# yuanming-hu/exposure

Measured on AMD Instinct MI355X. Metric: Mpixels/s through 8-step filter chain fwd+bwd, higher is better.
Workload: dtype f16; 1 GPU; 8-step filter chain (E,G,W,S+,T,Ct,BW,C) fwd+bwd, 64x512x512x3 f16 NHWC per GPU, one HIP kernel per filter step and direction; batch_per_gpu=64, global_batch=64, height=512, width=512, parallelism=image-sharded replicas x1 (no data-path collective), weak scaling, launch=hipGraph replay, 10 steps (330 captured launches) per replay, chain_streams=2, transport=none (one process)

## Files before the change

exposure_amd/csrc/exposure_hip.hip:

```cpp
#include <dlfcn.h>
#include <hip/hip_runtime.h>
#include <stdint.h>
#include <stdio.h>
#include <stdlib.h>
#include <string.h>
#include <mutex>
#include <vector>
#include <string>
#include <type_traits>

#include "../../include/exposure_hip.h"
#include "filter_math.h"
#include "pixel_io.h"
#include "kernel_common.h"
#include "host_common.h"
#include "stream_bodies.h"



namespace expo {


template <class F, typename T, bool VEC, class IO>
__global__ __launch_bounds__(kThreads) void filter_fwd_kernel(const T* __restrict__ x, T* __restrict__ y,
// ... 1388 lines not shown
  if (g.stream) hipLaunchKernelGGL((vignet_fwd_kernel<T, true, IoStream>), grid, block, 0, s, (const T*)x, (T*)y, mp, sharp, masking, h, w, g.groups);
  else if (g.vec) hipLaunchKernelGGL((vignet_fwd_kernel<T, true>), grid, block, 0, s, (const T*)x, (T*)y, mp, sharp, masking, h, w, g.groups);
  else hipLaunchKernelGGL((vignet_fwd_kernel<T, false>), grid, block, 0, s, (const T*)x, (T*)y, mp, sharp, masking, h, w, g.groups);
  HIP_TRY(hipGetLastError(), "vignet_fwd launch");
  return EXPO_OK;
}

template <typename T>
static int vignet_bwd_t(const void* x, const void* dy, void* dx, const float* mp, float* dmp, float sharp, int masking,
                        int n, int h, int w, void* workspace, size_t workspace_bytes, hipStream_t s) {
  const Geom g = make_geom<T>(n, h, w, {x, dy, dx}, kGeomApply);
  const dim3 grid(g.blocks_x, n), block(kThreads);
  float* records;
  if (int rc = ws_check(workspace, workspace_bytes, n, g.blocks_x, 1, &records)) return rc;
#define EXPO_L(VEC, HAS_DX, IO) \
  hipLaunchKernelGGL((vignet_bwd_kernel<T, VEC, HAS_DX, IO>), grid, block, 0, s, (const T*)x, (const T*)dy, (T*)dx, mp, records, sharp, masking, h, w, g.groups)
  if (g.vec) { if (dx) EXPO_L(true, true, IoCached); else EXPO_L(true, false, IoCached); }
  else { if (dx) EXPO_L(false, true, IoCached); else EXPO_L(false, false, IoCached); }
#undef EXPO_L
  HIP_TRY(hipGetLastError(), "vignet_bwd launch");
  FinishArgs fa{};
  fa.s[0] = FinishStep{mp, dmp, nullptr, records, nullptr, kFinVignet, 0, masking ? 1 : 0, sharp, g.blocks_x};
  return launch_finish(fa, 1, n, s);
}

template <typename T>
static int penalty_bwd_t(const void* y, const float* dpen, void* dy, int n, int h, int w, hipStream_t s) {
  const Geom g = make_geom<T>(n, h, w, {y, dy}, kGeomMap);
  const dim3 grid(g.blocks_x, n), block(kThreads);
  const float inv_count = 1.0f / (float(g.hw) * 3.0f);
#define EXPO_L(VEC, IO) \
  hipLaunchKernelGGL((penalty_bwd_kernel<T, VEC, IO>), grid, block, 0, s, (const T*)y, dpen, (T*)dy, g.hw, g.groups, inv_count)
  if (g.stream) EXPO_L(true, IoStream); else if (g.vec) EXPO_L(true, IoCached); else EXPO_L(false, IoCached);
#undef EXPO_L
  HIP_TRY(hipGetLastError(), "penalty_bwd launch");
  return EXPO_OK;
}

template <typename T>
static int stats_bwd_t(const void* x, const float* stats, const float* dstats, void* dx, int n, int h, int w,
                       hipStream_t s) {
  const Geom g = make_geom<T>(n, h, w, {x, dx}, kGeomMap);
  const dim3 grid(g.blocks_x, n), block(kThreads);
  const float inv_hw = 1.0f / float(g.hw);
#define EXPO_L(VEC, IO) \
  hipLaunchKernelGGL((stats_bwd_kernel<T, VEC, IO>), grid, block, 0, s, (const T*)x, stats, dstats, (T*)dx, g.hw, g.groups, inv_hw)
  if (g.stream) EXPO_L(true, IoStream); else if (g.vec) EXPO_L(true, IoCached); else EXPO_L(false, IoCached);
#undef EXPO_L
  HIP_TRY(hipGetLastError(), "stats_bwd launch");
  return EXPO_OK;
}

template <typename T>
static int stats_jvp_t(const void* x, const float* stats, const void* v, float* jv, int n, int h, int w,
                       void* workspace, size_t workspace_bytes, hipStream_t s) {
  const Geom g = make_geom<T>(n, h, w, {x, v}, kGeomReadReduce);
  const dim3 grid(g.blocks_x, n), block(kThreads);
  float* records;
  if (int rc = ws_check(workspace, workspace_bytes, n, g.blocks_x, 1, &records)) return rc;
#define EXPO_L(VEC, IO) \
  hipLaunchKernelGGL((stats_jvp_kernel<T, VEC, IO>), grid, block, 0, s, (const T*)x, stats, (const T*)v, records, g.hw, g.groups)
  if (g.stream) EXPO_L(true, IoStream); else if (g.vec) EXPO_L(true, IoCached); else EXPO_L(false, IoCached);
#undef EXPO_L
  HIP_TRY(hipGetLastError(), "stats_jvp launch");
  FinishArgs fa{};
  fa.s[0] = FinishStep{nullptr, jv, nullptr, records, nullptr, kFinScaled, 3, 0, 1.0f / float(g.hw), g.blocks_x};
  return launch_finish(fa, 1, n, s);
}

template <typename T>
static int stats_hvp_t(const void* x, const float* dstats, const float* jv, const void* v, void* out, int n, int h,
                       int w, hipStream_t s) {
  const Geom g = make_geom<T>(n, h, w, {x, v, out}, kGeomMap);
  const dim3 grid(g.blocks_x, n), block(kThreads);
  const float inv_hw = 1.0f / float(g.hw);
#define EXPO_L(VEC, IO) \
  hipLaunchKernelGGL((stats_hvp_kernel<T, VEC, IO>), grid, block, 0, s, (const T*)x, dstats, jv, (const T*)v, (T*)out, g.hw, g.groups, inv_hw)
  if (g.stream) EXPO_L(true, IoStream); else if (g.vec) EXPO_L(true, IoCached); else EXPO_L(false, IoCached);
#undef EXPO_L
  HIP_TRY(hipGetLastError(), "stats_hvp launch");
  return EXPO_OK;
}

}

using namespace expo;

struct ForkJoin {
  hipStream_t helper = nullptr;
  hipEvent_t fork = nullptr, join = nullptr;
};
__device__ int g_lane_probe[2];
__global__ void lane_probe_wait_kernel(int gen, long long limit_ticks) {
  if (threadIdx.x != 0) return;
  const long long t0 = wall_clock64();
  int seen = 0;
  do {
    seen = __hip_atomic_load(&g_lane_probe[0], __ATOMIC_RELAXED, __HIP_MEMORY_SCOPE_AGENT);
    if (seen == gen) break;
    __builtin_amdgcn_s_sleep(64);
  } while (wall_clock64() - t0 < limit_ticks);
  __hip_atomic_store(&g_lane_probe[1], seen == gen ? gen : -gen, __ATOMIC_RELAXED, __HIP_MEMORY_SCOPE_AGENT);
}
__global__ void lane_probe_set_kernel(int gen) {
  if (threadIdx.x == 0) __hip_atomic_store(&g_lane_probe[0], gen, __ATOMIC_RELAXED, __HIP_MEMORY_SCOPE_AGENT);
}
static int lanes_run_side_by_side(hipStream_t s, hipStream_t h) {
  static int gen = 0;
  ++gen;
  hipLaunchKernelGGL(lane_probe_wait_kernel, dim3(1), dim3(64), 0, s, gen, 50000LL);
  hipLaunchKernelGGL(lane_probe_set_kernel, dim3(1), dim3(64), 0, h, gen);
  if (hipGetLastError() != hipSuccess) return -1;
  if (hipStreamSynchronize(h) != hipSuccess || hipStreamSynchronize(s) != hipSuccess) return -1;
  int got[2] = {0, 0};
  if (hipMemcpyFromSymbol(got, HIP_SYMBOL(g_lane_probe), sizeof(got)) != hipSuccess) return -1;
  return got[1] == gen ? 1 : got[1] == -gen ? 0 : -1;
}
static int g_helper_probes = 0, g_helper_rejected = 0;

constexpr int kMaxProbeAttempts = 4;
constexpr size_t kMaxSpares = 8;
struct HelperEntry {
  int dev;
  hipStream_t caller;
  unsigned long long caller_id;
  ForkJoin fj;
  bool probed;
  std::mutex mu;
};
static std::vector<HelperEntry*> g_helper_table;
static std::vector<hipStream_t> g_helper_spares;
static std::mutex g_helper_mu;
static bool helper_probe_enabled() {
  static const bool probe = !(getenv("EXPO_CHAIN_HELPER_PROBE") && atoi(getenv("EXPO_CHAIN_HELPER_PROBE")) == 0);
  return probe;
}
static unsigned long long stream_id_of(hipStream_t s) {
  using GetId = hipError_t (*)(hipStream_t, unsigned long long*);
  static const GetId get_id = reinterpret_cast<GetId>(dlsym(RTLD_DEFAULT, "hipStreamGetId"));
  unsigned long long id = 0;
  if (!get_id) return 0;
  if (get_id(s, &id) != hipSuccess) {
    (void)hipGetLastError();
    id = 0;
  }
  return id;
}
static void park_or_destroy(hipStream_t st) {
  std::lock_guard<std::mutex> lock(g_helper_mu);
  if (g_helper_spares.size() < kMaxSpares)
    g_helper_spares.push_back(st);
  else
    (void)hipStreamDestroy(st);
}
static void probe_helper(HelperEntry* e) {
  hipStreamCaptureMode mode = hipStreamCaptureModeRelaxed;
  (void)hipThreadExchangeStreamCaptureMode(&mode);
  hipStream_t first = e->fj.helper, cand = first;
  bool found = false;
  for (int attempt = 0; attempt < kMaxProbeAttempts; ++attempt) {
    {
      std::lock_guard<std::mutex> lock(g_helper_mu);
      ++g_helper_probes;
    }
    const int r = lanes_run_side_by_side(e->caller, cand);
    if (r != 0) {
      found = true;
      break;
    }
    {
      std::lock_guard<std::mutex> lock(g_helper_mu);
      ++g_helper_rejected;
    }
    if (cand != first) park_or_destroy(cand);
    cand = nullptr;
    if (attempt + 1 == kMaxProbeAttempts) break;
    if (hipStreamCreateWithFlags(&cand, hipStreamNonBlocking) != hipSuccess) {
      (void)hipGetLastError();
      cand = nullptr;
      break;
    }
  }
  if (found && cand != first) {
    park_or_destroy(first);
    e->fj.helper = cand;
  }
  (void)hipThreadExchangeStreamCaptureMode(&mode);
  e->probed = true;
}

static HelperEntry* helper_entry(hipStream_t caller, bool probe_now) {
  int dev = 0;
  if (hipGetDevice(&dev) != hipSuccess || dev < 0) return nullptr;
  const unsigned long long id = stream_id_of(caller);
  HelperEntry* e = nullptr;
  {
    std::lock_guard<std::mutex> lock(g_helper_mu);
    for (HelperEntry* t : g_helper_table)
      if (t->dev == dev && t->caller == caller) e = t;
    if (e && e->caller_id != id) {
      e->caller_id = id;
      e->probed = !helper_probe_enabled();
    }
    if (!e) {
      hipStream_t st;
      hipEvent_t e0, e1;
      if (hipStreamCreateWithFlags(&st, hipStreamNonBlocking) != hipSuccess) return nullptr;
      if (hipEventCreateWithFlags(&e0, hipEventDisableTiming) != hipSuccess ||
          hipEventCreateWithFlags(&e1, hipEventDisableTiming) != hipSuccess) return nullptr;
      e = new HelperEntry{dev, caller, id, ForkJoin{st, e0, e1}, !helper_probe_enabled(), {}};
      g_helper_table.push_back(e);
    }
  }
  if (!probe_now) return e;
  std::lock_guard<std::mutex> lock(e->mu);
  if (e->probed) return e;
  hipStreamCaptureStatus cap = hipStreamCaptureStatusNone;
  if (hipStreamIsCapturing(caller, &cap) != hipSuccess) {
    (void)hipGetLastError();
    return e;
  }
  if (cap != hipStreamCaptureStatusNone) return e;
  probe_helper(e);
  return e;
}
static ForkJoin* fork_join_for_device(hipStream_t caller = nullptr) {
  HelperEntry* e = helper_entry(caller, true);
  return e ? &e->fj : nullptr;
}
static std::mutex g_fork_join_mu;
static int chain_fork(ForkJoin* fj, hipStream_t s) {
  std::lock_guard<std::mutex> lock(g_fork_join_mu);
  HIP_TRY(hipEventRecord(fj->fork, s), "chain fork");
  HIP_TRY(hipStreamWaitEvent(fj->helper, fj->fork, 0), "chain fork");
  return EXPO_OK;
}
static int chain_join(ForkJoin* fj, hipStream_t s) {
  std::lock_guard<std::mutex> lock(g_fork_join_mu);
  HIP_TRY(hipEventRecord(fj->join, fj->helper), "chain join");
  HIP_TRY(hipStreamWaitEvent(s, fj->join, 0), "chain join");
  return EXPO_OK;
}
static bool chain_split(int n, int h, int w, int dtype) {
  static const int forced = getenv("EXPO_CHAIN_STREAMS") ? atoi(getenv("EXPO_CHAIN_STREAMS")) : 0;
  if (n < 2) return false;
  if (forced == 1) return false;
  if (forced >= 2) return true;
  const long bytes = long(n) * h * w * 3L * (dtype == EXPO_F16 ? 2L : 4L);
  return bytes >= (40L << 20) && bytes < (256L << 20);
}

static bool chain_snake(int n, int h, int w, int dtype) {
  static const int forced = getenv("EXPO_CHAIN_SNAKE") ? atoi(getenv("EXPO_CHAIN_SNAKE")) : -1;
  if (forced >= 0) return forced != 0;
  const long bytes = long(n) * h * w * 3L * (dtype == EXPO_F16 ? 2L : 4L);
  return bytes >= (256L << 20);
}

struct ChainChunk { int nb, np, lane; };
struct ChainPlan {
  std::vector<ChainChunk> chunks;
  bool two_lanes = false, snake = false;
};
static ChainPlan chain_plan(int n, int h, int w, int dtype) {
  static const int tile_mib = getenv("EXPO_CHAIN_TILE_MIB") ? atoi(getenv("EXPO_CHAIN_TILE_MIB")) : 96;
  ChainPlan plan;
  const long image_bytes = long(h) * w * 3L * (dtype == EXPO_F16 ? 2L : 4L);
  const long bytes = long(n) * image_bytes;
  int tiles = 1;
  static const long tile_min = long(getenv("EXPO_CHAIN_TILE_MIN_MIB") ? atoi(getenv("EXPO_CHAIN_TILE_MIN_MIB")) : 256) << 20;
  if (tile_mib > 0 && bytes >= tile_min && n > 1) {
    long tile_n = (long(tile_mib) << 20) / image_bytes;
    if (tile_n < 1) tile_n = 1;
    tiles = int((n + tile_n - 1) / tile_n);
  }
  if (tiles == 1) {
    plan.snake = chain_snake(n, h, w, dtype);
    plan.two_lanes = chain_split(n, h, w, dtype);
    const int n0 = plan.two_lanes ? n / 2 : n;
    plan.chunks.push_back({0, n0, 0});
    if (plan.two_lanes) plan.chunks.push_back({n0, n - n0, 1});
    return plan;
  }
  const int base = n / tiles, rem = n % tiles;
  plan.two_lanes = chain_split(base, h, w, dtype);
  int at = 0;
  for (int t = 0; t < tiles; ++t) {
    const int tn = base + (t < rem ? 1 : 0);
    const int n0 = (plan.two_lanes && tn >= 2) ? tn / 2 : tn;
    plan.chunks.push_back({at, n0, 0});
    if (n0 < tn) plan.chunks.push_back({at + n0, tn - n0, 1});
    at += tn;
  }
  return plan;
}

static int chain_fuse_steps(const ChainPlan& plan) {
  static const int forced = env_int("EXPO_CHAIN_FUSE_STEPS", 0);
  if (plan.snake) return 1;
  const int k = forced > 0 ? forced : kChainFuseMax;
  return k < kChainFuseMax ? k : kChainFuseMax;
}

extern "C" {

int expo_version(void) { return EXPO_ABI_VERSION; }

const char* expo_last_error(void) { return g_err.c_str(); }

#ifndef EXPO_SOURCE_DIGEST
#define EXPO_SOURCE_DIGEST "unknown"
#endif
const char* expo_build_info(void) { return EXPO_SOURCE_DIGEST; }

int expo_num_filter_params(int filter_id) {
  if (filter_id < 0 || filter_id >= EXPO_NUM_FILTERS) return -1;
  return kNumParams[filter_id];
}

size_t expo_workspace_bytes(int n, int h, int w, int dtype) {
  if (check_common(n, h, w, dtype) != EXPO_OK || n == 0) return 0;
  const int bx = geom_bx_max(n, h, w, dtype);
  return ws_step_bytes(n, bx);
}

int expo_filter_fwd(int filter_id, const void* x, void* y, const float* params, int n, int h, int w, int dtype,
                    void* stream) {
  if (int rc = check_common(n, h, w, dtype)) return rc;
  if (filter_id < 0 || filter_id >= EXPO_NUM_FILTERS) return fail(EXPO_E_BADARG, "filter_id out of range");
  if (n == 0) return EXPO_OK;
  if (!x || !y || !params) return fail(EXPO_E_BADARG, "null pointer");
  hipStream_t s = static_cast<hipStream_t>(stream);
  return dtype == EXPO_F16 ? fwd_by_id<half_t>(filter_id, x, y, params, n, h, w, s)
                           : fwd_by_id<float>(filter_id, x, y, params, n, h, w, s);
}

static int filter_bwd_common(int filter_id, const void* x, const void* dy, void* dx, const float* params,
                             float* dparams, int n, int h, int w, int dtype, int hsv_grad_mode, void* workspace,
                             size_t workspace_bytes, void* stream, bool accum) {
  if (int rc = check_common(n, h, w, dtype)) return rc;
  if (filter_id < 0 || filter_id >= EXPO_NUM_FILTERS) return fail(EXPO_E_BADARG, "filter_id out of range");
  if (hsv_grad_mode != 0 && hsv_grad_mode != 1) return fail(EXPO_E_BADARG, "hsv_grad_mode must be 0 or 1");
  if (n == 0) return EXPO_OK;
  if (!x || !dy || !params || !dparams) return fail(EXPO_E_BADARG, "null pointer");
  hipStream_t s = static_cast<hipStream_t>(stream);
  const int bx = geom_bx(bwd_geom_kind(filter_id), n, h, w, dtype);
  float* records;
  if (int rc = ws_check(workspace, workspace_bytes, n, bx, 1, &records)) return rc;
  const int rc = dtype == EXPO_F16
                     ? bwd_by_id<half_t>(filter_id, x, dy, dx, params, records, n, h, w, hsv_grad_mode, s)
                     : bwd_by_id<float>(filter_id, x, dy, dx, params, records, n, h, w, hsv_grad_mode, s);
  if (rc) return rc;
  FinishArgs fa{};
  fa.s[0] = FinishStep{params, dparams, nullptr, records, nullptr, kFinFilter, filter_id, accum ? 1 : 0, 0.f, bx};
  return launch_finish(fa, 1, n, s);
}

int expo_filter_bwd(int filter_id, const void* x, const void* dy, void* dx, const float* params, float* dparams,
                    int n, int h, int w, int dtype, int hsv_grad_mode, void* workspace, size_t workspace_bytes,
                    void* stream) {
  return filter_bwd_common(filter_id, x, dy, dx, params, dparams, n, h, w, dtype, hsv_grad_mode, workspace,
                           workspace_bytes, stream, false);
}

int expo_filter_bwd_accumulate(int filter_id, const void* x, const void* dy, void* dx, const float* params,
                               float* dparams, int n, int h, int w, int dtype, int hsv_grad_mode, void* workspace,
                               size_t workspace_bytes, void* stream) {
  return filter_bwd_common(filter_id, x, dy, dx, params, dparams, n, h, w, dtype, hsv_grad_mode, workspace,
                           workspace_bytes, stream, true);
}

int expo_filter_apply_fwd(int filter_id, const void* x, void* y, const float* params, const float* mask_params,
                          float maximum_sharpness, float minimum_strength, int n, int h, int w, int dtype,
                          void* stream) {
  if (int rc = check_common(n, h, w, dtype)) return rc;
  if (filter_id < 0 || filter_id >= EXPO_NUM_FILTERS) return fail(EXPO_E_BADARG, "filter_id out of range");
  if (n == 0) return EXPO_OK;
  if (!x || !y || !params || !mask_params) return fail(EXPO_E_BADARG, "null pointer");
  hipStream_t s = static_cast<hipStream_t>(stream);
  return dtype == EXPO_F16 ? apply_fwd_by_id<half_t>(filter_id, x, y, params, mask_params, maximum_sharpness,
                                                     minimum_strength, n, h, w, s)
                           : apply_fwd_by_id<float>(filter_id, x, y, params, mask_params, maximum_sharpness,
                                                    minimum_strength, n, h, w, s);
}

int expo_filter_apply_bwd(int filter_id, const void* x, const void* dy, void* dx, const float* params,
                          float* dparams, const float* mask_params, float* dmask_params, float maximum_sharpness,
                          float minimum_strength, int n, int h, int w, int dtype, int hsv_grad_mode, void* workspace,
                          size_t workspace_bytes, void* stream) {
  if (int rc = check_common(n, h, w, dtype)) return rc;
  if (filter_id < 0 || filter_id >= EXPO_NUM_FILTERS) return fail(EXPO_E_BADARG, "filter_id out of range");
  if (hsv_grad_mode != 0 && hsv_grad_mode != 1) return fail(EXPO_E_BADARG, "hsv_grad_mode must be 0 or 1");
  if (n == 0) return EXPO_OK;
  if (!x || !dy || !params || !dparams || !mask_params || !dmask_params) return fail(EXPO_E_BADARG, "null pointer");
  hipStream_t s = static_cast<hipStream_t>(stream);
  const int bx = geom_bx(kGeomApply, n, h, w, dtype);
  float* records;
  if (int rc = ws_check(workspace, workspace_bytes, n, bx, 1, &records)) return rc;
  const int rc = dtype == EXPO_F16
                     ? apply_bwd_by_id<half_t>(filter_id, x, dy, dx, params, mask_params, records, maximum_sharpness,
                                               minimum_strength, n, h, w, hsv_grad_mode, s)
                     : apply_bwd_by_id<float>(filter_id, x, dy, dx, params, mask_params, records, maximum_sharpness,
                                              minimum_strength, n, h, w, hsv_grad_mode, s);
  if (rc) return rc;
  FinishArgs fa{};
  fa.s[0] = FinishStep{params, dparams, dmask_params, records, nullptr, kFinApply, filter_id, 0, 0.f, bx};
  return launch_finish(fa, 1, n, s);
}

int expo_filter_apply_dispatch_fwd(const int32_t* filter_ids, const void* x, void* y, const float* params,
                                   const float* mask_params, float maximum_sharpness, float minimum_strength, int n,
                                   int h, int w, int dtype, void* stream) {
  if (int rc = check_common(n, h, w, dtype)) return rc;
  if (n == 0) return EXPO_OK;
  if (!filter_ids || !x || !y || !params || !mask_params) return fail(EXPO_E_BADARG, "null pointer");
  hipStream_t s = static_cast<hipStream_t>(stream);
  return dtype == EXPO_F16 ? apply_dispatch_fwd_t<half_t>(filter_ids, x, y, params, mask_params, maximum_sharpness,
                                                          minimum_strength, n, h, w, s)
                           : apply_dispatch_fwd_t<float>(filter_ids, x, y, params, mask_params, maximum_sharpness,
                                                         minimum_strength, n, h, w, s);
}

int expo_filter_apply_dispatch_bwd(const int32_t* filter_ids, const void* x, const void* dy, void* dx,
                                   const float* params, float* dparams, const float* mask_params, float* dmask_params,
                                   float maximum_sharpness, float minimum_strength, int n, int h, int w, int dtype,
                                   int hsv_grad_mode, void* workspace, size_t workspace_bytes, void* stream) {
  if (int rc = check_common(n, h, w, dtype)) return rc;
  if (hsv_grad_mode != 0 && hsv_grad_mode != 1) return fail(EXPO_E_BADARG, "hsv_grad_mode must be 0 or 1");
  if (n == 0) return EXPO_OK;
  if (!filter_ids || !x || !dy || !params || !dparams || !mask_params || !dmask_params)
    return fail(EXPO_E_BADARG, "null pointer");
  hipStream_t s = static_cast<hipStream_t>(stream);
  return dtype == EXPO_F16
             ? apply_dispatch_bwd_t<half_t>(filter_ids, x, dy, dx, params, dparams, mask_params, dmask_params,
                                            maximum_sharpness, minimum_strength, n, h, w, hsv_grad_mode, workspace,
                                            workspace_bytes, s)
             : apply_dispatch_bwd_t<float>(filter_ids, x, dy, dx, params, dparams, mask_params, dmask_params,
                                           maximum_sharpness, minimum_strength, n, h, w, hsv_grad_mode, workspace,
                                           workspace_bytes, s);
}

int expo_filter_dispatch_fwd(const int32_t* filter_ids, const void* x, void* y, const float* params,
                             float* penalty, int n, int h, int w, int dtype, void* workspace,
                             size_t workspace_bytes, void* stream) {
  if (int rc = check_common(n, h, w, dtype)) return rc;
  if (n == 0) return EXPO_OK;
  if (!filter_ids || !x || !y || !params) return fail(EXPO_E_BADARG, "null pointer");
  hipStream_t s = static_cast<hipStream_t>(stream);
  return dtype == EXPO_F16
             ? dispatch_fwd_t<half_t>(filter_ids, x, y, params, penalty, n, h, w, workspace, workspace_bytes, s)
             : dispatch_fwd_t<float>(filter_ids, x, y, params, penalty, n, h, w, workspace, workspace_bytes, s);
}

int expo_filter_dispatch_bwd(const int32_t* filter_ids, const void* x, const void* dy, void* dx,
                             const float* params, float* dparams, const float* dpenalty, int n, int h, int w,
                             int dtype, int hsv_grad_mode, void* workspace, size_t workspace_bytes, void* stream) {
  if (int rc = check_common(n, h, w, dtype)) return rc;
  if (hsv_grad_mode != 0 && hsv_grad_mode != 1) return fail(EXPO_E_BADARG, "hsv_grad_mode must be 0 or 1");
  if (n == 0) return EXPO_OK;
  if (!filter_ids || !x || !dy || !params || !dparams) return fail(EXPO_E_BADARG, "null pointer");
  hipStream_t s = static_cast<hipStream_t>(stream);
  return dtype == EXPO_F16 ? dispatch_bwd_t<half_t>(filter_ids, x, dy, dx, params, dparams, dpenalty, n, h, w,
                                                    hsv_grad_mode, workspace, workspace_bytes, s)
                           : dispatch_bwd_t<float>(filter_ids, x, dy, dx, params, dparams, dpenalty, n, h, w,
                                                   hsv_grad_mode, workspace, workspace_bytes, s);
}

int expo_chain_streams(int n, int h, int w, int dtype) {
  if (check_common(n, h, w, dtype) != EXPO_OK) return 0;
  return chain_plan(n, h, w, dtype).two_lanes ? 2 : 1;
}

int expo_chain_plan(int n, int h, int w, int dtype, int* chunks, int max_chunks, int* lanes, int* snake) {
  if (int rc = check_common(n, h, w, dtype)) return rc;
  if (max_chunks < 0 || (max_chunks > 0 && !chunks)) return fail(EXPO_E_BADARG, "bad chunk buffer");
  if (n == 0) return 0;
  const ChainPlan plan = chain_plan(n, h, w, dtype);
  for (size_t c = 0; c < plan.chunks.size() && int(c) < max_chunks; ++c) {
    chunks[3 * c] = plan.chunks[c].nb;
    chunks[3 * c + 1] = plan.chunks[c].np;
    chunks[3 * c + 2] = plan.chunks[c].lane;
  }
  if (lanes) *lanes = plan.two_lanes ? 2 : 1;
  if (snake) *snake = plan.snake ? 1 : 0;
  return int(plan.chunks.size());
}

int expo_chain_prepare(void* stream) {
  return helper_entry(static_cast<hipStream_t>(stream), true) ? EXPO_OK : fail(EXPO_E_HIP, "chain helper stream");
}

int expo_chain_release(void* stream) {
  int dev = 0;
  HIP_TRY(hipGetDevice(&dev), "hipGetDevice");
  HelperEntry* found = nullptr;
  {
    std::lock_guard<std::mutex> lock(g_helper_mu);
    for (size_t i = 0; i < g_helper_table.size(); ++i)
      if (g_helper_table[i]->dev == dev && g_helper_table[i]->caller == static_cast<hipStream_t>(stream)) {
        found = g_helper_table[i];
        g_helper_table.erase(g_helper_table.begin() + i);
        break;
      }
  }
  if (!found) return EXPO_OK;
  {
    std::lock_guard<std::mutex> lock(found->mu);
    (void)hipStreamSynchronize(found->fj.helper);
    (void)hipEventDestroy(found->fj.fork);
    (void)hipEventDestroy(found->fj.join);
    (void)hipStreamDestroy(found->fj.helper);
  }
  delete found;
  return EXPO_OK;
}

int expo_chain_helper_stats(int* probed, int* rejected) {
  if (probed) *probed = g_helper_probes;
  if (rejected) *rejected = g_helper_rejected;
  return EXPO_OK;
}

int expo_chain_fwd(const int* filter_ids, int steps, void* const* acts, const float* const* params, int n, int h,
                   int w, int dtype, void* stream) {
  if (steps < 0 || !filter_ids || !acts || !params) return fail(EXPO_E_BADARG, "bad chain arguments");
  if (int rc = check_common(n, h, w, dtype)) return rc;
  if (n == 0) return EXPO_OK;
  hipStream_t s = static_cast<hipStream_t>(stream);
  for (int i = 0; i < steps; ++i) {
    if (filter_ids[i] < 0 || filter_ids[i] >= EXPO_NUM_FILTERS) return fail(EXPO_E_BADARG, "filter_id out of range");
    if (!acts[i] || !acts[i + 1] || !params[i]) return fail(EXPO_E_BADARG, "null pointer");
  }
  const size_t esz = dtype == EXPO_F16 ? 2 : 4;
  const ChainPlan plan = chain_plan(n, h, w, dtype);
  ForkJoin* fj = plan.two_lanes ? fork_join_for_device(s) : nullptr;
  if (plan.two_lanes && !fj) return fail(EXPO_E_HIP, "helper stream unavailable");
  if (fj) {
    if (int rc = chain_fork(fj, s)) return rc;
  }
  int rc = EXPO_OK;
  const int fuse = chain_steps_vec_path(acts, steps, h, w, dtype) ? chain_fuse_steps(plan) : 1;
  for (size_t c = 0; c < plan.chunks.size() && !rc; ++c) {
    const ChainChunk& ck = plan.chunks[c];
    hipStream_t sp = ck.lane ? fj->helper : s;
    const size_t ioff = size_t(ck.nb) * h * w * 3 * esz;
    int cnt = 1;
    for (int i = 0; i < steps && !rc; i += cnt) {
      cnt = steps - i < fuse ? steps - i : fuse;
      if (cnt > 1) {
        rc = chain_steps_fwd(filter_ids + i, cnt, acts + i, params + i, ck.nb, ck.np, h, w, dtype, n, sp);
      } else {
        const int rev = plan.snake ? (i & 1) : 0;
        const void* xin = static_cast<const char*>(acts[i]) + ioff;
        void* yout = static_cast<char*>(acts[i + 1]) + ioff;
        const float* prm = params[i] + size_t(ck.nb) * kNumParams[filter_ids[i]];
        rc = dtype == EXPO_F16 ? fwd_by_id<half_t>(filter_ids[i], xin, yout, prm, ck.np, h, w, sp, rev, n)
                               : fwd_by_id<float>(filter_ids[i], xin, yout, prm, ck.np, h, w, sp, rev, n);
      }
    }
  }
  if (fj) {
    const int jrc = chain_join(fj, s);
    if (!rc) rc = jrc;
  }
  return rc;
}

int expo_filter_bwd_records(int filter_id, const void* x, const void* dy, void* dx, const float* params, int n,
                            int h, int w, int dtype, int hsv_grad_mode, void* records, size_t records_bytes,
                            void* stream) {
  if (int rc = check_common(n, h, w, dtype)) return rc;
  if (filter_id < 0 || filter_id >= EXPO_NUM_FILTERS) return fail(EXPO_E_BADARG, "filter_id out of range");
  if (hsv_grad_mode != 0 && hsv_grad_mode != 1) return fail(EXPO_E_BADARG, "hsv_grad_mode must be 0 or 1");
  if (n == 0) return EXPO_OK;
  if (!x || !dy || !params) return fail(EXPO_E_BADARG, "null pointer");
  hipStream_t s = static_cast<hipStream_t>(stream);
  const int bx = geom_bx(bwd_geom_kind(filter_id), n, h, w, dtype);
  float* rec;
  if (int rc = ws_check(records, records_bytes, n, bx, 1, &rec)) return rc;
  return dtype == EXPO_F16 ? bwd_by_id<half_t>(filter_id, x, dy, dx, params, rec, n, h, w, hsv_grad_mode, s)
                           : bwd_by_id<float>(filter_id, x, dy, dx, params, rec, n, h, w, hsv_grad_mode, s);
}

int expo_finish_bwd(const int* filter_ids, int steps, const float* const* params, float* const* dparams, int n,
                    int h, int w, int dtype, void* workspace, size_t workspace_bytes, void* stream) {
  if (steps < 0 || !filter_ids || !params || !dparams) return fail(EXPO_E_BADARG, "bad finish arguments");
  if (int rc = check_common(n, h, w, dtype)) return rc;
  if (n == 0 || steps == 0) return EXPO_OK;
  hipStream_t s = static_cast<hipStream_t>(stream);
  const int bx_max = geom_bx_max(n, h, w, dtype);
  float* records;
  if (int rc = ws_check(workspace, workspace_bytes, n, bx_max, steps, &records)) return rc;
  const size_t step_floats = ws_step_bytes(n, bx_max) / sizeof(float);
  for (int i = 0; i < steps; ++i) {
    if (filter_ids[i] < 0 || filter_ids[i] >= EXPO_NUM_FILTERS) return fail(EXPO_E_BADARG, "filter_id out of range");
    if (!params[i] || !dparams[i]) return fail(EXPO_E_BADARG, "null pointer");
  }
  for (int i0 = 0; i0 < steps; i0 += kMaxFinishSteps) {
    const int cnt = steps - i0 < kMaxFinishSteps ? steps - i0 : kMaxFinishSteps;
    FinishArgs fa{};
    for (int k = 0; k < cnt; ++k)
      fa.s[k] = FinishStep{params[i0 + k], dparams[i0 + k], nullptr, records + size_t(i0 + k) * step_floats, nullptr,
                           kFinFilter, filter_ids[i0 + k], 0, 0.f,
                           geom_bx(bwd_geom_kind(filter_ids[i0 + k]), n, h, w, dtype)};
    if (int rc = launch_finish(fa, cnt, n, s)) return rc;
  }
  return EXPO_OK;
}

int expo_chain_bwd(const int* filter_ids, int steps, void* const* acts, void* const* grads,
                   const float* const* params, float* const* dparams, int n, int h, int w, int dtype,
                   int hsv_grad_mode, void* workspace, size_t workspace_bytes, void* stream) {
  if (steps < 0 || !filter_ids || !acts || !grads || !params || !dparams)
    return fail(EXPO_E_BADARG, "bad chain arguments");
  if (int rc = check_common(n, h, w, dtype)) return rc;
  if (hsv_grad_mode != 0 && hsv_grad_mode != 1) return fail(EXPO_E_BADARG, "hsv_grad_mode must be 0 or 1");
  if (n == 0 || steps == 0) return EXPO_OK;
  hipStream_t s = static_cast<hipStream_t>(stream);
  for (int i = 0; i < steps; ++i) {
    if (filter_ids[i] < 0 || filter_ids[i] >= EXPO_NUM_FILTERS) return fail(EXPO_E_BADARG, "filter_id out of range");
    if (!dparams[i] || !acts[i] || !grads[i + 1] || !params[i]) return fail(EXPO_E_BADARG, "null pointer");
  }
  const int bx_max = geom_bx_max(n, h, w, dtype);
  float* records;
  if (int rc = ws_check(workspace, workspace_bytes, n, bx_max, steps, &records)) return rc;
  const size_t step_floats = ws_step_bytes(n, bx_max) / sizeof(float);
  const size_t esz = dtype == EXPO_F16 ? 2 : 4;
  const ChainPlan plan = chain_plan(n, h, w, dtype);
  ForkJoin* fj = plan.two_lanes ? fork_join_for_device(s) : nullptr;
  if (plan.two_lanes && !fj) return fail(EXPO_E_HIP, "helper stream unavailable");
  if (fj) {
    if (int rc = chain_fork(fj, s)) return rc;
  }
  int rc = EXPO_OK;
  for (size_t c = 0; c < plan.chunks.size() && !rc; ++c) {
    const ChainChunk& ck = plan.chunks[c];
    hipStream_t sp = ck.lane ? fj->helper : s;
    const size_t ioff = size_t(ck.nb) * h * w * 3 * esz;
    for (int i = steps - 1; i >= 0 && !rc; --i) {
      const int rev = plan.snake ? ((i + 1) & 1) : 0;
      const int bx = geom_bx(bwd_geom_kind(filter_ids[i]), n, h, w, dtype);
      float* rec = records + size_t(i) * step_floats + size_t(ck.nb) * bx * kWsSlots;
      const void* xin = static_cast<const char*>(acts[i]) + ioff;
      const void* gin = static_cast<const char*>(grads[i + 1]) + ioff;
      void* gout = grads[i] ? static_cast<char*>(grads[i]) + ioff : nullptr;
      const float* prm = params[i] + size_t(ck.nb) * kNumParams[filter_ids[i]];
      rc = dtype == EXPO_F16
               ? bwd_by_id<half_t>(filter_ids[i], xin, gin, gout, prm, rec, ck.np, h, w, hsv_grad_mode, sp, rev, n)
               : bwd_by_id<float>(filter_ids[i], xin, gin, gout, prm, rec, ck.np, h, w, hsv_grad_mode, sp, rev, n);
    }
  }
  if (fj) {
    const int jrc = chain_join(fj, s);
    if (!rc) rc = jrc;
  }
  if (rc) return rc;
  return expo_finish_bwd(filter_ids, steps, params, dparams, n, h, w, dtype, workspace, workspace_bytes, stream);
}

int expo_critic_stats(const void* x, float* stats, int n, int h, int w, int dtype, void* workspace,
                      size_t workspace_bytes, void* stream) {
  if (int rc = check_common(n, h, w, dtype)) return rc;
  if (n == 0) return EXPO_OK;
  if (!x || !stats) return fail(EXPO_E_BADARG, "null pointer");
  hipStream_t s = static_cast<hipStream_t>(stream);
  return dtype == EXPO_F16 ? stats_t<half_t>(x, stats, n, h, w, workspace, workspace_bytes, s)
                           : stats_t<float>(x, stats, n, h, w, workspace, workspace_bytes, s);
}

int expo_overexposure_penalty(const void* y, float* penalty, int n, int h, int w, int dtype, void* workspace,
                              size_t workspace_bytes, void* stream) {
  if (int rc = check_common(n, h, w, dtype)) return rc;
  if (n == 0) return EXPO_OK;
  if (!y || !penalty) return fail(EXPO_E_BADARG, "null pointer");
  hipStream_t s = static_cast<hipStream_t>(stream);
  return dtype == EXPO_F16 ? penalty_t<half_t>(y, penalty, n, h, w, workspace, workspace_bytes, s)
                           : penalty_t<float>(y, penalty, n, h, w, workspace, workspace_bytes, s);
}

int expo_vignet_apply_fwd(const void* x, void* y, const float* mask_params, float maximum_sharpness, int masking, int n,
                          int h, int w, int dtype, void* stream) {
  if (int rc = check_common(n, h, w, dtype)) return rc;
  if (n == 0) return EXPO_OK;
  if (!x || !y || !mask_params) return fail(EXPO_E_BADARG, "null pointer");
  hipStream_t s = static_cast<hipStream_t>(stream);
  return dtype == EXPO_F16 ? vignet_fwd_t<half_t>(x, y, mask_params, maximum_sharpness, masking, n, h, w, s)
                           : vignet_fwd_t<float>(x, y, mask_params, maximum_sharpness, masking, n, h, w, s);
}

int expo_vignet_apply_bwd(const void* x, const void* dy, void* dx, const float* mask_params, float* dmask_params,
                          float maximum_sharpness, int masking, int n, int h, int w, int dtype, void* workspace,
                          size_t workspace_bytes, void* stream) {
  if (int rc = check_common(n, h, w, dtype)) return rc;
  if (n == 0) return EXPO_OK;
  if (!x || !dy || !mask_params || !dmask_params) return fail(EXPO_E_BADARG, "null pointer");
  hipStream_t s = static_cast<hipStream_t>(stream);
  return dtype == EXPO_F16 ? vignet_bwd_t<half_t>(x, dy, dx, mask_params, dmask_params, maximum_sharpness, masking, n, h,
                                                  w, workspace, workspace_bytes, s)
                           : vignet_bwd_t<float>(x, dy, dx, mask_params, dmask_params, maximum_sharpness, masking, n, h,
                                                 w, workspace, workspace_bytes, s);
}

int expo_overexposure_penalty_bwd(const void* y, const float* dpenalty, void* dy, int n, int h, int w, int dtype,
                                  void* stream) {
  if (int rc = check_common(n, h, w, dtype)) return rc;
  if (n == 0) return EXPO_OK;
  if (!y || !dpenalty || !dy) return fail(EXPO_E_BADARG, "null pointer");
  hipStream_t s = static_cast<hipStream_t>(stream);
  return dtype == EXPO_F16 ? penalty_bwd_t<half_t>(y, dpenalty, dy, n, h, w, s)
                           : penalty_bwd_t<float>(y, dpenalty, dy, n, h, w, s);
}

int expo_critic_stats_bwd(const void* x, const float* stats, const float* dstats, void* dx, int n, int h, int w,
                          int dtype, void* stream) {
  if (int rc = check_common(n, h, w, dtype)) return rc;
  if (n == 0) return EXPO_OK;
  if (!x || !stats || !dstats || !dx) return fail(EXPO_E_BADARG, "null pointer");
  hipStream_t s = static_cast<hipStream_t>(stream);
  return dtype == EXPO_F16 ? stats_bwd_t<half_t>(x, stats, dstats, dx, n, h, w, s)
                           : stats_bwd_t<float>(x, stats, dstats, dx, n, h, w, s);
}

int expo_critic_stats_jvp(const void* x, const float* stats, const void* v, float* jv, int n, int h, int w, int dtype,
                          void* workspace, size_t workspace_bytes, void* stream) {
  if (int rc = check_common(n, h, w, dtype)) return rc;
  if (n == 0) return EXPO_OK;
  if (!x || !stats || !v || !jv) return fail(EXPO_E_BADARG, "null pointer");
  hipStream_t s = static_cast<hipStream_t>(stream);
  return dtype == EXPO_F16 ? stats_jvp_t<half_t>(x, stats, v, jv, n, h, w, workspace, workspace_bytes, s)
                           : stats_jvp_t<float>(x, stats, v, jv, n, h, w, workspace, workspace_bytes, s);
}

int expo_critic_penalty_tangent(const float* u, const float* x, const float* stats, float scale, float* t0, float* norm,
                                float* term, int n, int h, int w, void* stream) {
  if (int rc = check_common(n, h, w, EXPO_F32)) return rc;
  if (n == 0) return EXPO_OK;
  if (!u || !x || !stats || !t0 || !norm || !term) return fail(EXPO_E_BADARG, "null pointer");
  if (long(h) * w > (1L << 24)) return fail(EXPO_E_BADARG, "critic_penalty_tangent: at most 2^24 pixels per image");
  if (h * w <= 4096 && (reinterpret_cast<uintptr_t>(u) & 7) == 0 && (reinterpret_cast<uintptr_t>(t0) & 7) == 0)
    hipLaunchKernelGGL(critic_penalty_tangent_reg_kernel, dim3(n), dim3(1024), 0, static_cast<hipStream_t>(stream), u, x, stats,
                       scale, t0, norm, term, h * w);
  else
    hipLaunchKernelGGL(critic_penalty_tangent_kernel, dim3(n), dim3(1024), 0, static_cast<hipStream_t>(stream), u, x, stats,
                       scale, t0, norm, term, h * w);
  HIP_TRY(hipGetLastError(), "critic_penalty_tangent launch");
  return EXPO_OK;
}

int expo_net_inputs(const void* a, const int64_t* a_rows, const void* b, const int64_t* b_rows, const float* alpha,
                    const float* vec_a, const float* vec_b, int v0, float* planes, float* stats, float* x_out, int x_first,
                    int x_count, int n, int h, int w, int dtype, float offset, void* stream) {
  if (int rc = check_common(n, h, w, dtype)) return rc;
  if (n == 0) return EXPO_OK;
  if (!a || !b || !planes || !stats) return fail(EXPO_E_BADARG, "null pointer");
  if (long(h) * w > kNetInputsMaxPixels) return fail(EXPO_E_BADARG, "net_inputs: at most 4096 pixels per image (the image is held in LDS)");
  if (v0 < 0 || v0 > 58) return fail(EXPO_E_BADARG, "net_inputs: 0 <= v0 <= 58");
  if (v0 > 0 && (!vec_a || !vec_b)) return fail(EXPO_E_BADARG, "net_inputs: v0 > 0 needs vec_a and vec_b");
  if (v0 > 0 && alpha) return fail(EXPO_E_BADARG, "net_inputs: the interpolated block takes no per-image values");
  const int m = (alpha ? 3 : 2) * n;
  if (x_out && (x_first < 0 || x_count < 0 || x_first + x_count > m)) return fail(EXPO_E_BADARG, "net_inputs: x rows outside the batch");
  NetInputsArgs g{a, b, reinterpret_cast<const long long*>(a_rows), reinterpret_cast<const long long*>(b_rows), alpha, vec_a, vec_b,
                  planes, stats, x_out, n, h * w, v0, x_first, x_out ? x_count : 0, offset,
                  unsigned((0x100000000ull + (6 + v0) - 1) / (6 + v0))};
  int parts = (256 + m / 2) / m;
  const int max_parts = (h * w * (6 + v0) + 1023) / 1024;
  if (parts > max_parts) parts = max_parts;
  if (parts > 16) parts = 16;
  if (parts < 1) parts = 1;
  const dim3 grid(m, parts);
  hipStream_t s = static_cast<hipStream_t>(stream);
  if (dtype == EXPO_F16) hipLaunchKernelGGL((net_inputs_kernel<half_t, 1024>), grid, dim3(1024), 0, s, g);
  else hipLaunchKernelGGL((net_inputs_kernel<float, 1024>), grid, dim3(1024), 0, s, g);
  HIP_TRY(hipGetLastError(), "net_inputs launch");
  return EXPO_OK;
}

int expo_critic_stats_hvp(const void* x, const float* dstats, const float* jv, const void* v, void* out, int n, int h,
                          int w, int dtype, void* stream) {
  if (int rc = check_common(n, h, w, dtype)) return rc;
  if (n == 0) return EXPO_OK;
  if (!x || !dstats || !jv || !v || !out) return fail(EXPO_E_BADARG, "null pointer");
  hipStream_t s = static_cast<hipStream_t>(stream);
  return dtype == EXPO_F16 ? stats_hvp_t<half_t>(x, dstats, jv, v, out, n, h, w, s)
                           : stats_hvp_t<float>(x, dstats, jv, v, out, n, h, w, s);
}

}
#endif
```

exposure_amd/csrc/host_common.h:

```cpp
#pragma once
#include <hip/hip_runtime.h>
#include <stdint.h>
#include <stdlib.h>

#include <initializer_list>
#include <string>

#include "../../include/exposure_hip.h"
#include "kernel_common.h"

namespace expo {

extern thread_local std::string g_err;

inline int fail(int code, const char* what) {
  g_err = what;
  return code;
}
inline int fail_hip(hipError_t e, const char* where) {
  g_err = std::string(where) + ": " + hipGetErrorString(e);
  return EXPO_E_HIP;
}
#define HIP_TRY(expr, where)                         \
  do {                                               \
    hipError_t e_ = (expr);                          \
    if (e_ != hipSuccess) return fail_hip(e_, where); \
  } while (0)

constexpr int kNumParams[EXPO_NUM_FILTERS] = {1, 1, 3, 1, 8, 1, 1, 24, 2};

struct Geom {
  int hw, groups, blocks_x;
  bool vec;
  bool stream;
};

inline int env_int(const char* name, int dflt) {
  const char* v = getenv(name);
  if (!v || !*v) return dflt;
  const int x = atoi(v);
  return x > 0 ? x : dflt;
}

inline long stream_min_bytes() {
  static const long v = env_int("EXPO_STREAM_MIN_BYTES", 8 << 20);
  return v;
}

constexpr int kMaxReduceBlocksX = 1024;
enum GeomKind {
  kGeomMap = 0,
  kGeomReduce = 1,
  kGeomReadReduce = 2,
  kGeomDispatch = 3,
  kGeomReduceTone = 4,
  kGeomReduceColor = 5,
  kGeomApply = 6,
  kGeomFusedBwd = 7,
  kNumGeomKinds = 8
};
inline int bwd_geom_kind(int filter_id) { return filter_id == 4 ? kGeomReduceTone : filter_id == 7 ? kGeomReduceColor : kGeomReduce; }

template <typename T>
inline Geom make_geom(int n, int h, int w, std::initializer_list<const void*> ptrs, int kind) {
  const bool reduces = kind != kGeomMap;
  constexpr int PPL = PixTraits<T>::PPL;
  Geom g;
  g.hw = h * w;
  g.groups = (g.hw + PPL - 1) / PPL;
  g.vec = (g.hw % VecTraits<T>::PPV) == 0;
  for (const void* p : ptrs) g.vec = g.vec && (p == nullptr || (reinterpret_cast<uintptr_t>(p) & 3) == 0);
  const int max_bx = (g.groups + kThreads - 1) / kThreads;
  static const int gpt_kind[kNumGeomKinds] = {
      env_int("EXPO_FWD_GROUPS_PER_THREAD", 1),       env_int("EXPO_BWD_GROUPS_PER_THREAD", 1),
      env_int("EXPO_RED_GROUPS_PER_THREAD", 4),       env_int("EXPO_DISPATCH_GROUPS_PER_THREAD", 4),
      env_int("EXPO_TONE_GROUPS_PER_THREAD", 2),      env_int("EXPO_COLOR_GROUPS_PER_THREAD", 2),
      env_int("EXPO_APPLY_GROUPS_PER_THREAD", 4),     env_int("EXPO_FUSED_BWD_GROUPS_PER_THREAD", 8)};
  int gpt = gpt_kind[kind >= 0 && kind < kNumGeomKinds ? kind : kGeomReduce];
  static const bool bwd_gpt_forced = getenv("EXPO_BWD_GROUPS_PER_THREAD") != nullptr;
  if (kind == kGeomReduce && !bwd_gpt_forced && long(n) * g.hw * 3L * long(sizeof(T)) >= (256L << 20) && gpt < 4) gpt = 4;
  int bx = (g.groups + kThreads * gpt - 1) / (kThreads * gpt);
  const long want = 1024;
  if (long(bx) * n < want) bx = int((want + n - 1) / n);
  if (bx > max_bx) bx = max_bx;
  if (reduces && bx > kMaxReduceBlocksX) bx = kMaxReduceBlocksX;
  if (bx < 1) bx = 1;
  g.blocks_x = bx;
  g.stream = g.vec && long(n) * g.hw * 3L * long(sizeof(T)) >= stream_min_bytes();
  return g;
}

int chain_records(void* workspace, size_t workspace_bytes, int n, int h, int w, int dtype, int steps, float** records,
                  size_t* step_floats);
int finish_chain_fused(const int32_t* ids, const float* params, float* dparams, const float* records,
                       size_t step_floats, int steps, int n, int blocks_x, hipStream_t s);

constexpr int kChainFuseMax = 8;
bool chain_steps_vec_path(void* const* acts, int steps, int h, int w, int dtype);
int chain_steps_fwd(const int* ids, int cnt, void* const* acts, const float* const* params, int nb, int np, int h,
                    int w, int dtype, int n_geom, hipStream_t s);

inline int check_common(int n, int h, int w, int dtype) {
  if (n < 0 || h < 1 || w < 1) return fail(EXPO_E_BADARG, "n >= 0, h >= 1, w >= 1 required");
  if (n > 65535) return fail(EXPO_E_BADARG, "n > 65535 not supported (grid.y)");
  if (dtype != EXPO_F16 && dtype != EXPO_F32) return fail(EXPO_E_BADDTYPE, "dtype must be EXPO_F16 or EXPO_F32");
  const long image_bytes = long(h) * long(w) * 3L * (dtype == EXPO_F16 ? 2L : 4L);
  if (image_bytes > (1L << 31) - 8192) return fail(EXPO_E_BADARG, "one image must be smaller than 2 GiB");
  return EXPO_OK;
}

}
```

Before: 31950 Mpixels/s.

## Fuse runs of element-wise backward filter steps into one multi-step kernel

Adds a backward kernel that walks a run of consecutive element-wise filters (exposure, gamma, white balance, saturation, level) in one pass. The upstream gradient is read once and carried in registers through each step, and every step's dx and parameter-gradient partials are still written. Per-step accumulators live in LDS and each step is block-reduced into its own record slot at the end. The aim is to cut intermediate gradient re-reads and kernel launches in the backward chain. The cost is higher register and LDS pressure from holding one activation tile per fused step, and extra code instantiations for each run length.

```diff
diff --git a/exposure_amd/csrc/chain_steps_bwd.hip b/exposure_amd/csrc/chain_steps_bwd.hip
--- /dev/null
+++ b/exposure_amd/csrc/chain_steps_bwd.hip
@@ -0,0 +1,214 @@
+#include <hip/hip_runtime.h>
+#include <stdint.h>
+
+#include "../../include/exposure_hip.h"
+#include "filter_math.h"
+#include "pixel_io.h"
+#include "kernel_common.h"
+#include "host_common.h"
+#include "stream_bodies.h"
+
+namespace expo {
+
+template <int NS>
+struct ChainStepsBwdArgs {
+  const void* dy;
+  const void* x[NS];
+  void* dx[NS];
+  const float* prm[NS];
+  float* rec[NS];
+  int id[NS];
+  int acc_at[NS];
+  int acc_floats, hw;
+};
+
+template <class F, typename T, int MODE>
+__device__ __forceinline__ void run_step(const float* prm, const RawGroup& x, RawGroup& g, float* lds) {
+  constexpr int PPL = PixTraits<T>::PPL;
+  constexpr int kParts = kAccParts < PPL ? kAccParts : PPL;
+  static_assert(!F::kHasGroupBwd && F::kLutFloats == 0, "element-wise filters only");
+  const typename F::Prm q = F::load(prm);
+  float a[kParts][F::NACC];
+#pragma unroll
+  for (int p = 0; p < kParts; ++p)
+#pragma unroll
+    for (int j = 0; j < F::NACC; ++j) a[p][j] = lds[(p * F::NACC + j) * kThreads];
+  float v[PPL * 3], d[PPL * 3];
+  unpack<T>(x, v);
+  unpack<T>(g, d);
+#pragma unroll
+  for (int k = 0; k < PPL; ++k) {
+    float dx[3];
+    F::bwd(q, nullptr, v + 3 * k, d + 3 * k, dx, a[k % kParts], MODE);
+#pragma unroll
+    for (int c = 0; c < 3; ++c) d[3 * k + c] = dx[c];
+  }
+  g = pack<T>(d);
+#pragma unroll
+  for (int p = 0; p < kParts; ++p)
+#pragma unroll
+    for (int j = 0; j < F::NACC; ++j) lds[(p * F::NACC + j) * kThreads] = a[p][j];
+}
+
+template <class F, typename T>
+__device__ __forceinline__ void run_reduce(const float* lds, float* rec) {
+  constexpr int PPL = PixTraits<T>::PPL;
+  constexpr int kParts = kAccParts < PPL ? kAccParts : PPL;
+  float acc[F::NACC];
+#pragma unroll
+  for (int j = 0; j < F::NACC; ++j) acc[j] = lds[j * kThreads];
+#pragma unroll
+  for (int p = 0; p < kParts - 1; ++p)
+#pragma unroll
+    for (int j = 0; j < F::NACC; ++j) acc[j] += lds[((p + 1) * F::NACC + j) * kThreads];
+  block_reduce_record<F::NACC>(acc, rec);
+}
+
+#define EXPO_RUN_FILTERS(X) X(0, ExposureF) X(1, GammaF) X(2, WhiteBalanceF) X(3, SatPlusF) X(8, LevelF)
+
+bool chain_steps_bwd_fusable(int id, int dtype, int mode) {
+  if (id == 3 && dtype == EXPO_F32 && mode == 1) return false;
+  return chain_steps_bwd_acc_floats(id) > 0;
+}
+
+int chain_steps_bwd_acc_floats(int id) {
+  switch (id) {
+#define EXPO_CASE(ID, F) \
+  case ID: return kAccParts * F::NACC;
+    EXPO_RUN_FILTERS(EXPO_CASE)
+#undef EXPO_CASE
+  }
+  return 0;
+}
+
+template <typename T, int MODE, class IO, int NS>
+__global__ __launch_bounds__(kThreads EXPO_BWD_MIN_WAVES) void chain_steps_bwd_kernel(const ChainStepsBwdArgs<NS> a) {
+  constexpr int PPL = PixTraits<T>::PPL;
+  static_assert(PPL >= kAccParts, "kParts == kAccParts in both storage types");
+  const int n = blockIdx.y;
+  const int hw = a.hw;
+  const size_t off = size_t(n) * hw * 3;
+  const int lane = threadIdx.x & 63;
+#if EXPO_FP16_OVFL
+  if constexpr (sizeof(T) == 2) __builtin_amdgcn_s_setreg(1 | (23 << 6) | (0 << 11), 1);
+#endif
+  const int stride = gridDim.x * kThreads;
+  int gw = blockIdx.x * kThreads + (threadIdx.x & ~63);
+  const bool work = gw * PPL < hw;
+  const __amdgpu_buffer_rsrc_t rdy = make_image_rsrc(static_cast<const T*>(a.dy) + off, hw);
+  int boff = chunk_byte_offset<T>(gw, lane);
+  RawGroup cur, x[NS];
+  if (work) {
+    cur = load_raw<IO::kLoadDy>(rdy, boff);
+#pragma unroll
+    for (int k = 0; k < NS; ++k)
+      x[k] = load_raw<IO::kLoadX>(make_image_rsrc(static_cast<const T*>(a.x[k]) + off, hw), boff);
+  }
+  extern __shared__ float accs[];
+  float* const mine = accs + threadIdx.x;
+  for (int f = 0; f < a.acc_floats; ++f) mine[f * kThreads] = 0.f;
+  if (work) {
+    while (true) {
+      const int gn = gw + stride;
+      const bool more = gn * PPL < hw;
+      const int bnext = chunk_byte_offset<T>(gn, lane);
+      RawGroup nxt = cur;
+      if (more) nxt = load_raw<IO::kLoadDy>(rdy, bnext);
+#pragma unroll 1
+      for (int st = 0; st < NS; ++st) {
+        const float* const prm = a.prm[st];
+        float* const lds = mine + a.acc_at[st] * kThreads;
+#define EXPO_CASE(ID, F) \
+  case ID: run_step<F, T, MODE>(prm + n * F::NP, x[0], cur, lds); break;
+        switch (a.id[st]) {
+          EXPO_RUN_FILTERS(EXPO_CASE)
+          default: break;
+        }
+#undef EXPO_CASE
+        store_raw<IO::kStore>(make_image_rsrc(static_cast<T*>(a.dx[st]) + off, hw), boff, cur);
+#pragma unroll
+        for (int k = 0; k + 1 < NS; ++k) x[k] = x[k + 1];
+        if (more) x[NS - 1] = load_raw<IO::kLoadX>(make_image_rsrc(static_cast<const T*>(a.x[st]) + off, hw), bnext);
+      }
+      if (!more) break;
+      gw = gn;
+      boff = bnext;
+      cur = nxt;
+    }
+  }
+#pragma unroll 1
+  for (int st = 0; st < NS; ++st) {
+    if (st > 0) __syncthreads();
+    float* const rec = a.rec[st] + size_t(n) * gridDim.x * kWsSlots;
+    const float* const lds = mine + a.acc_at[st] * kThreads;
+#define EXPO_CASE(ID, F) \
+  case ID: run_reduce<F, T>(lds, rec); break;
+    switch (a.id[st]) {
+      EXPO_RUN_FILTERS(EXPO_CASE)
+      default: break;
+    }
+#undef EXPO_CASE
+  }
+}
+
+template <typename T, int MODE, int NS>
+static int chain_steps_bwd_launch(const ChainStepsBwdArgs<NS>& a, const Geom& g, int np, hipStream_t s) {
+  const dim3 grid(g.blocks_x, np), block(kThreads);
+  const size_t lds = size_t(a.acc_floats) * kThreads * sizeof(float);
+  if (g.stream)
+    hipLaunchKernelGGL((chain_steps_bwd_kernel<T, MODE, IoStream, NS>), grid, block, lds, s, a);
+  else
+    hipLaunchKernelGGL((chain_steps_bwd_kernel<T, MODE, IoCached, NS>), grid, block, lds, s, a);
+  HIP_TRY(hipGetLastError(), "chain_steps_bwd launch");
+  return EXPO_OK;
+}
+
+template <typename T, int NS>
+static int chain_steps_bwd_t(const int* ids, int i0, void* const* acts, void* const* grads,
+                             const float* const* params, float* records, size_t step_floats, int nb, int np, int h,
+                             int w, int mode, int n_geom, hipStream_t s) {
+  const Geom g = make_geom<T>(n_geom, h, w, {}, kGeomReduce);
+  const size_t ioff = size_t(nb) * h * w * 3 * sizeof(T);
+  ChainStepsBwdArgs<NS> a{};
+  a.dy = static_cast<const char*>(grads[i0 + 1]) + ioff;
+  for (int k = 0; k < NS; ++k) {
+    const int i = i0 - k;
+    a.x[k] = static_cast<const char*>(acts[i]) + ioff;
+    a.dx[k] = static_cast<char*>(grads[i]) + ioff;
+    a.prm[k] = params[i] + size_t(nb) * kNumParams[ids[i]];
+    a.rec[k] = records + size_t(i) * step_floats + size_t(nb) * g.blocks_x * kWsSlots;
+    a.id[k] = ids[i];
+    a.acc_at[k] = a.acc_floats;
+    a.acc_floats += chain_steps_bwd_acc_floats(ids[i]);
+  }
+  a.hw = h * w;
+  return mode == 1 ? chain_steps_bwd_launch<T, 1, NS>(a, g, np, s) : chain_steps_bwd_launch<T, 0, NS>(a, g, np, s);
+}
+
+int chain_steps_bwd(const int* ids, int i0, int cnt, void* const* acts, void* const* grads,
+                    const float* const* params, float* records, size_t step_floats, int nb, int np, int h, int w,
+                    int dtype, int mode, int n_geom, hipStream_t s) {
+  if (cnt < 2 || cnt > kChainFuseMax || cnt > i0 + 1) return fail(EXPO_E_BADARG, "chain_steps_bwd: step count");
+  int acc_floats = 0;
+  for (int k = 0; k < cnt; ++k) {
+    if (!chain_steps_bwd_fusable(ids[i0 - k], dtype, mode) || !grads[i0 - k])
+      return fail(EXPO_E_BADARG, "chain_steps_bwd: not a step of the run table with a dx");
+    acc_floats += chain_steps_bwd_acc_floats(ids[i0 - k]);
+  }
+  if (acc_floats > kChainBwdAccFloatsMax) return fail(EXPO_E_BADARG, "chain_steps_bwd: accumulators of the run");
+#define EXPO_GO(NS)                                                                                                   \
+  case NS:                                                                                                            \
+    return dtype == EXPO_F16                                                                                          \
+               ? chain_steps_bwd_t<half_t, NS>(ids, i0, acts, grads, params, records, step_floats, nb, np, h, w, mode, \
+                                               n_geom, s)                                                             \
+               : chain_steps_bwd_t<float, NS>(ids, i0, acts, grads, params, records, step_floats, nb, np, h, w, mode,  \
+                                              n_geom, s);
+  switch (cnt) {
+    EXPO_GO(2) EXPO_GO(3) EXPO_GO(4) EXPO_GO(5) EXPO_GO(6) EXPO_GO(7) EXPO_GO(8)
+  }
+#undef EXPO_GO
+  static_assert(kChainFuseMax == 8, "one instantiation per run length");
+  return fail(EXPO_E_BADARG, "chain_steps_bwd: step count");
+}
+
+}
diff --git a/exposure_amd/csrc/exposure_hip.hip b/exposure_amd/csrc/exposure_hip.hip
--- a/exposure_amd/csrc/exposure_hip.hip
+++ b/exposure_amd/csrc/exposure_hip.hip
@@ -1714,6 +1714,13 @@
   return k < kChainFuseMax ? k : kChainFuseMax;
 }
 
+static int chain_fuse_bwd_steps(const ChainPlan& plan) {
+  static const int forced = env_int("EXPO_CHAIN_FUSE_BWD_STEPS", 0);
+  if (plan.snake) return 1;
+  const int k = forced > 0 ? forced : kChainFuseMax;
+  return k < kChainFuseMax ? k : kChainFuseMax;
+}
+
 extern "C" {
 
 int expo_version(void) { return EXPO_ABI_VERSION; }
@@ -2045,11 +2052,32 @@
     if (int rc = chain_fork(fj, s)) return rc;
   }
   int rc = EXPO_OK;
+  int fuse = chain_steps_vec_path(acts, steps - 1, h, w, dtype) ? chain_fuse_bwd_steps(plan) : 1;
+  for (int i = 0; i <= steps && fuse > 1; ++i)
+    if ((reinterpret_cast<uintptr_t>(grads[i]) & 3) != 0) fuse = 1;
+  auto run_from = [&](int i) {
+    int cnt = 0, acc_floats = 0;
+    while (cnt < fuse && i - cnt >= 0) {
+      const int id = filter_ids[i - cnt];
+      if (!chain_steps_bwd_fusable(id, dtype, hsv_grad_mode) || !grads[i - cnt]) break;
+      acc_floats += chain_steps_bwd_acc_floats(id);
+      if (acc_floats > kChainBwdAccFloatsMax) break;
+      ++cnt;
+    }
+    return cnt > 1 ? cnt : 1;
+  };
   for (size_t c = 0; c < plan.chunks.size() && !rc; ++c) {
     const ChainChunk& ck = plan.chunks[c];
     hipStream_t sp = ck.lane ? fj->helper : s;
     const size_t ioff = size_t(ck.nb) * h * w * 3 * esz;
-    for (int i = steps - 1; i >= 0 && !rc; --i) {
+    int cnt = 1;
+    for (int i = steps - 1; i >= 0 && !rc; i -= cnt) {
+      cnt = fuse > 1 ? run_from(i) : 1;
+      if (cnt > 1) {
+        rc = chain_steps_bwd(filter_ids, i, cnt, acts, grads, params, records, step_floats, ck.nb, ck.np, h, w, dtype,
+                             hsv_grad_mode, n, sp);
+        continue;
+      }
       const int rev = plan.snake ? ((i + 1) & 1) : 0;
       const int bx = geom_bx(bwd_geom_kind(filter_ids[i]), n, h, w, dtype);
       float* rec = records + size_t(i) * step_floats + size_t(ck.nb) * bx * kWsSlots;
diff --git a/exposure_amd/csrc/host_common.h b/exposure_amd/csrc/host_common.h
--- a/exposure_amd/csrc/host_common.h
+++ b/exposure_amd/csrc/host_common.h
@@ -99,6 +99,12 @@
 bool chain_steps_vec_path(void* const* acts, int steps, int h, int w, int dtype);
 int chain_steps_fwd(const int* ids, int cnt, void* const* acts, const float* const* params, int nb, int np, int h,
                     int w, int dtype, int n_geom, hipStream_t s);
+constexpr int kChainBwdAccFloatsMax = 48;
+int chain_steps_bwd_acc_floats(int id);
+bool chain_steps_bwd_fusable(int id, int dtype, int mode);
+int chain_steps_bwd(const int* ids, int i0, int cnt, void* const* acts, void* const* grads,
+                    const float* const* params, float* records, size_t step_floats, int nb, int np, int h, int w,
+                    int dtype, int mode, int n_geom, hipStream_t s);
 
 inline int check_common(int n, int h, int w, int dtype) {
   if (n < 0 || h < 1 || w < 1) return fail(EXPO_E_BADARG, "n >= 0, h >= 1, w >= 1 required");
```

Measured after the change: 34120 Mpixels/s, median of 6. 6.8% higher.
